# maxwellsh/DIGDriver

Hardware: NVIDIA B200
Metric: genome_bases_scanned_per_s (higher is better)
Workload: dtype u8 bases -> int32 counts; f64 p-values

## Files before the change

### digdriver_b200/_lib.py

```python
import ctypes
import os

_PKG_DIR = os.path.dirname(os.path.abspath(__file__))
LIB_PATH = os.environ.get("DIG_LIB_PATH") or os.path.join(_PKG_DIR, "libdigb200.so")

_c = ctypes
_P = _c.c_void_p
_I64 = _c.c_int64
_I = _c.c_int
_U64 = _c.c_uint64
_D = _c.c_double

SIGNATURES = {
    "dig_version": (_I, []),
    "dig_last_error": (_c.c_char_p, []),
    "dig_device_sm_count": (_I, []),
    "dig_packed_words": (_I64, [_I64]),
    "dig_nmask_words": (_I64, [_I64]),
    "dig_pack_genome": (_I, [_P, _I64, _P, _P, _P, _P]),
    "dig_scan_workspace_bytes": (_I64, [_I64]),
    "dig_count_contexts": (_I, [_P, _P, _I64, _P, _P, _P, _P, _P, _P, _I64, _I, _I, _P, _P, _P, _P]),
    "dig_count_contexts_fused53": (_I, [_P, _P, _I64, _P, _P, _P, _P, _P, _I64, _P, _P, _P, _P, _P, _P]),
    "dig_narrow_counts_u16": (_I, [_P, _I64, _P, _P, _P]),
    "dig_peer_broadcast": (_I, [_P, _I64, _P, _I, _P]),
    "dig_nmask_fill_runs": (_I, [_P, _I64, _P, _I64, _I64, _P]),
    "dig_nmask_summary": (_I, [_P, _I64, _I64, _P, _P]),
    "dig_tabulate_capacity": (_I64, [_I64]),
    "dig_tabulate_elements_workspace_bytes": (_I64, [_I64]),
    "dig_tabulate_genes_workspace_bytes": (_I64, [_I64]),
    "dig_synth_genome": (_I, [_P, _I64, _I64, _U64, _I, _P]),
    "dig_mutation_contexts": (_I, [_P, _P, _I64, _P, _P, _P, _P, _P, _I64, _I, _I, _P, _P]),
    "dig_substitution_counts": (_I, [_P, _P, _I64, _I, _I, _P, _P]),
    "dig_count_hits": (_I, [_P, _P, _P, _P, _I64, _P, _P, _I64, _P, _P]),
    "dig_tabulate_elements": (_I, [_P, _P, _P, _P, _I64, _P, _P, _P, _P, _I64, _P, _P, _P, _I64, _I64, _P,
                                   _I64, _I64, _I64, _P, _P, _I, _P]),
    "dig_site_counts": (_I, [_P, _P, _I64, _I64, _I, _P, _P]),
    "dig_tabulate_genes": (_I, [_P, _P, _P, _I64, _P, _P, _I64, _I64, _I64, _P, _P, _P, _P]),
    "dig_element_transfer": (_I, [_P, _P, _P, _P, _P, _I64, _I64, _I, _P, _P, _P, _P, _P, _P, _P, _I64, _I, _P,
                                  _P, _P, _I, _I, _P, _P, _P, _P, _P, _P, _P, _P, _P, _P]),
    "dig_nb_pvalue_greater_midp": (_I, [_P, _P, _P, _I64, _P, _P]),
    "dig_nb_burden_test": (_I, [_P, _P, _P, _P, _I64, _P, _P, _P]),
    "dig_fisher_combine2": (_I, [_P, _P, _I64, _P, _P]),
    "dig_sequence_freq": (_I, [_P, _P, _I, _P, _P]),
    "dig_size_ratio": (_I, [_P, _P, _I64, _P, _P]),
    "dig_gene_scale_sums": (_I, [_P, _P, _P, _P, _P, _P, _I64, _I64, _P, _P]),
    "dig_gene_burden_test": (_I, [_P, _P, _P, _P, _P, _P, _I64, _P, _D, _D, _P, _P]),
    "dig_gene_dnds_sel": (_I, [_P, _P, _P, _P, _I64, _P, _P]),
    "dig_selection_coefficient": (_I, [_P, _P, _P, _P, _P, _I64, _P, _P, _P]),
    "dig_window_denominators": (_I, [_P, _P, _I64, _P, _P, _P]),
    "dig_site_test": (_I, [_P, _P, _P, _P, _P, _I64, _I64, _I, _P, _P, _P, _P, _P, _P, _P, _D, _P, _P, _P, _P, _P]),
    "dig_region_prob_norm": (_I, [_P, _P, _I64, _I, _P, _P]),
    "dig_position_obs": (_I, [_P, _I64, _P, _P, _P, _P, _P, _I64, _I, _I, _I, _P, _I64, _P, _P]),
    "dig_position_test": (_I, [_P, _P, _I64, _P, _P, _P, _P, _P, _I64, _I, _I, _P, _P, _P, _P, _I, _P, _P, _P, _P,
                               _P, _P, _P]),
    "dig_nb_pvalue_exact": (_I, [_P, _P, _P, _I64, _P, _P]),
    "dig_nb_pvalue_variant": (_I, [_I, _P, _P, _P, _P, _I64, _P, _P]),
    "dig_loglik": (_I, [_I, _P, _P, _P, _I64, _P, _P]),
    "dig_gene_llr_test": (_I, [_I, _P, _P, _P, _P, _P, _P, _I64, _P, _P]),
    "dig_element_region_counts": (_I, [_P, _P, _P, _P, _P, _I64, _I64, _I, _P, _P, _P, _I64, _I, _P, _P, _P, _P]),
    "dig_element_psum": (_I, [_P, _P, _P, _I64, _P, _P, _P]),
    "dig_overlap_count": (_I, [_P, _P, _P, _I64, _P, _P, _I64, _P, _P]),
    "dig_overlap_fill": (_I, [_P, _P, _P, _I64, _P, _P, _I64, _P, _P, _P, _P]),
    "dig_cds_substitution_table": (_I, [_P, _P, _I64, _P, _P, _I, _P, _P, _P, _P, _P, _I64, _P, _I, _P, _I, _P, _P,
                                        _P, _P]),
    "dig_annotate_snvs": (_I, [_P, _P, _I64, _P, _P, _I, _P, _P, _P, _P, _P, _I64, _P, _I, _P, _I, _P, _P, _P, _P,
                               _I64, _P, _P, _P]),
}



class ScanOpts(ctypes.Structure):
    _fields_ = [("workspace_d", _c.c_void_p), ("workspace_bytes", _c.c_int64), ("variant", _c.c_int32),
                ("totals_limit_kb", _c.c_uint32), ("tile_window", _c.c_int64), ("n_peer_counts3", _c.c_int32),
                ("nsum_offset_words", _c.c_int32), ("peer_counts3_d", _c.c_void_p * 8), ("mc_counts3_d", _c.c_void_p)]


SCAN_AUTO, SCAN_PER_BASE, SCAN_HEX_PLAIN, SCAN_HEX = 0, 1, 2, 3

_lib = None

KERNELS_PER_CALL = {
    "dig_pack_genome": 1, "dig_count_contexts": 1, "dig_count_contexts_fused53": 1, "dig_synth_genome": 1, "dig_mutation_contexts": 1,
    "dig_substitution_counts": 1, "dig_count_hits": 1, "dig_tabulate_elements": 3, "dig_tabulate_genes": 2, "dig_site_counts": 1,
    "dig_element_transfer": 1, "dig_nb_pvalue_greater_midp": 1, "dig_nb_burden_test": 1, "dig_fisher_combine2": 1,
    "dig_sequence_freq": 1, "dig_size_ratio": 1, "dig_gene_scale_sums": 1, "dig_gene_burden_test": 2,
    "dig_window_denominators": 1, "dig_site_test": 1, "dig_gene_dnds_sel": 1, "dig_selection_coefficient": 1, "dig_region_prob_norm": 1, "dig_position_obs": 1, "dig_position_test": 1, "dig_nb_pvalue_exact": 1,
    "dig_nb_pvalue_variant": 1, "dig_loglik": 1, "dig_gene_llr_test": 1, "dig_overlap_count": 1, "dig_overlap_fill": 1,
    "dig_element_region_counts": 1, "dig_element_psum": 1, "dig_narrow_counts_u16": 1, "dig_peer_broadcast": 1, "dig_nmask_fill_runs": 1,
    "dig_nmask_summary": 1, "dig_cds_substitution_table": 1, "dig_annotate_snvs": 1,
}
launch_count = 0


class DigError(RuntimeError):
    pass


def load():
    global _lib
    if _lib is not None:
        return _lib
    if not os.path.exists(LIB_PATH):
        raise DigError(
            "libdigb200.so not found at %s: the CUDA extension is required (no CPU fallback). "
            "Build it with `python -m digdriver_b200.build`." % LIB_PATH)
    lib = ctypes.CDLL(LIB_PATH)
    for name, (res, args) in SIGNATURES.items():
        fn = getattr(lib, name)
        fn.restype = res
        fn.argtypes = args
    _lib = lib
    return lib


def check(rc, what=""):
    if rc != 0:
        msg = load().dig_last_error()
        raise DigError("%s failed with code %d: %s" % (what or "libdigb200 call", rc, (msg or b"").decode()))


def call(name, *args):
    global launch_count
    fn = getattr(load(), name)
    check(fn(*args), name)
    launch_count += KERNELS_PER_CALL.get(name, 0)
```

### digdriver_b200/csrc/mutctx.cu

```cuda
#include "dig_common.cuh"

namespace {

__global__ void __launch_bounds__(256) mutctx_kernel(
    const uint32_t *__restrict__ p2, const uint32_t *__restrict__ nmask, int64_t last_p, int64_t last_m,
    const int64_t *__restrict__ chrom_off, const int64_t *__restrict__ chrom_len,
    const int32_t *__restrict__ mut_chrom, const int64_t *__restrict__ mut_start,
    const uint8_t *__restrict__ mut_ref, int64_t n_mut, int n_up, int n_down, int32_t *__restrict__ ctx_out)
{
    const int klen = n_up + n_down + 1;
    const int64_t stride = (int64_t)gridDim.x * blockDim.x;
    for (int64_t i = (int64_t)blockIdx.x * blockDim.x + threadIdx.x; i < n_mut; i += stride) {
        const int32_t c = mut_chrom[i];
        const int64_t p = mut_start[i];
        const int64_t L = __ldg(chrom_len + c);
        const int64_t off = __ldg(chrom_off + c);
        int32_t ctx = -1;
        if (p - n_up >= 0 && p + n_down < L) {
            const int64_t f = off + p - n_up;
            const int64_t w = f >> 4, m = f >> 5;
            const unsigned long long pk = ((unsigned long long)__ldg(p2 + w) << 32) | __ldg(p2 + (w < last_p ? w + 1 : last_p));
            const unsigned long long mk = ((unsigned long long)__ldg(nmask + m) << 32) | __ldg(nmask + (m < last_m ? m + 1 : last_m));
            const uint32_t key = (uint32_t)(pk >> (64 - 2 * ((int)(f & 15) + klen))) & ((1u << (2 * klen)) - 1u);
            const uint32_t bad = (uint32_t)(mk >> (64 - ((int)(f & 31) + klen))) & ((1u << klen) - 1u);
            const uint32_t base = (key >> (2 * n_down)) & 3u;
            const bool base_n = ((bad >> n_down) & 1u) != 0u;
            auto mismatch = [&](int64_t row) -> bool {
                const uint32_t ref = mut_ref[row];
                return ref > 3u || base_n || base != ref;
            };
            bool dropped = mismatch(i);
            for (int64_t j = i - 1; !dropped && j >= 0 && mut_chrom[j] == c && mut_start[j] == p; --j)
                dropped = mismatch(j);
            if (!dropped && bad == 0u) ctx = (int32_t)key;
        }
        ctx_out[i] = ctx;
    }
}

__global__ void __launch_bounds__(256) subst_hist_kernel(const int32_t *__restrict__ ctx,
                                                         const uint8_t *__restrict__ alt, int64_t n, int n_down,
                                                         int n_bins, unsigned long long *__restrict__ counts)
{
    extern __shared__ unsigned int sh[];
    for (int k = threadIdx.x; k < n_bins; k += blockDim.x) sh[k] = 0u;
    __syncthreads();
    const int64_t stride = (int64_t)gridDim.x * blockDim.x;
    for (int64_t i = (int64_t)blockIdx.x * blockDim.x + threadIdx.x; i < n; i += stride) {
        const int32_t c = ctx[i];
        const uint32_t a = alt[i];
        if (c < 0 || a > 3u) continue;
        const uint32_t ref = ((uint32_t)c >> (2 * n_down)) & 3u;
        if (a == ref) continue;
        atomicAdd(sh + 3 * c + (int)(a > ref ? a - 1u : a), 1u);
    }
    __syncthreads();
    for (int k = threadIdx.x; k < n_bins; k += blockDim.x)
        if (sh[k]) atomicAdd(counts + k, (unsigned long long)sh[k]);
}

}

extern "C" int dig_substitution_counts(const int32_t *ctx_d, const uint8_t *alt_d, int64_t n, int n_up, int n_down,
                                       unsigned long long *counts_d, void *stream)
{
    DIG_CHECK_ARG(n >= 0, "negative size");
    DIG_CHECK_ARG(n_up >= 0 && n_down >= 0 && n_up + n_down <= 5, "unsupported context size");
    DIG_CHECK_ARG(counts_d != nullptr, "null pointer");
    const int n_bins = 3 << (2 * (n_up + n_down + 1));
    cudaStream_t st = (cudaStream_t)stream;
    DIG_CUDA(cudaMemsetAsync(counts_d, 0, (size_t)n_bins * sizeof(unsigned long long), st));
    if (n == 0) return DIG_OK;
    DIG_CHECK_ARG(ctx_d && alt_d, "null pointer");
    int64_t blocks = (n + 255) / 256;
    const int64_t cap = (int64_t)dig::sm_count() * 4;
    if (blocks > cap) blocks = cap;
    subst_hist_kernel<<<(unsigned)blocks, 256, (size_t)n_bins * sizeof(unsigned int), st>>>(ctx_d, alt_d, n, n_down,
                                                                                          n_bins, counts_d);
    DIG_CHECK_LAUNCH();
    return DIG_OK;
}

extern "C" int dig_mutation_contexts(const uint32_t *packed2_d, const uint32_t *nmask_d, int64_t n_bases,
                                     const int64_t *chrom_off_d, const int64_t *chrom_len_d,
                                     const int32_t *mut_chrom_d, const int64_t *mut_start_d,
                                     const uint8_t *mut_ref_d, int64_t n_mut, int n_up, int n_down,
                                     int32_t *ctx_out_d, void *stream)
{
    DIG_CHECK_ARG(n_mut >= 0 && n_bases >= 0, "negative size");
    DIG_CHECK_ARG(n_up >= 0 && n_down >= 0 && n_up + n_down <= 14, "unsupported context size");
    if (n_mut == 0) return DIG_OK;
    DIG_CHECK_ARG(packed2_d && nmask_d && chrom_off_d && chrom_len_d && mut_chrom_d && mut_start_d && mut_ref_d &&
                      ctx_out_d,
                  "null pointer");
    int64_t blocks = (n_mut + 255) / 256;
    const int64_t cap = (int64_t)dig::sm_count() * 32;
    if (blocks > cap) blocks = cap;
    mutctx_kernel<<<(unsigned)blocks, 256, 0, (cudaStream_t)stream>>>(
        packed2_d, nmask_d, (((n_bases + 31) >> 5) << 1) - 1, ((n_bases + 31) >> 5) - 1, chrom_off_d, chrom_len_d,
        mut_chrom_d, mut_start_d, mut_ref_d, n_mut, n_up, n_down, ctx_out_d);
    DIG_CHECK_LAUNCH();
    return DIG_OK;
}
```

### digdriver_b200/kernels.py

```python
import numpy as np
import torch

from . import _lib


def _stream(device, stream=None):
    st = stream if stream is not None else torch.cuda.current_stream(device)
    return st.cuda_stream


def _dev(x, dtype, device):
    if isinstance(x, torch.Tensor):
        return x.to(device=device, dtype=dtype).contiguous()
    return torch.from_numpy(np.ascontiguousarray(x)).to(device=device, dtype=dtype)


def _ptr(t):
    return t.data_ptr() if t is not None else None


def _tile_hint(reg_start, reg_end, tile_window):
    if tile_window is not None:
        return int(tile_window)
    if isinstance(reg_start, torch.Tensor) or isinstance(reg_end, torch.Tensor):
        return 0
    s, e = np.asarray(reg_start), np.asarray(reg_end)
    if s.size == 0:
        return 0
    w = int(e.flat[0]) - int(s.flat[0])
    return w if w > 0 and bool(np.all(e - s == w)) else 0


def _scan_opts(dev, n_reg, variant, totals_limit_kb, workspace, tile_window=0, peer_rows=None, mc_rows=None, genome=None):
    import ctypes
    if workspace is None and n_reg > 0:
        nbytes = int(_lib.load().dig_scan_workspace_bytes(int(n_reg)))
        workspace = torch.empty(nbytes, dtype=torch.uint8, device=dev)
    opts = _lib.ScanOpts(workspace.data_ptr() if workspace is not None else None,
                         workspace.numel() if workspace is not None else 0, int(variant), int(totals_limit_kb),
                         int(tile_window))
    if peer_rows:
        assert len(peer_rows) <= 8, "at most 8 peers"
        opts.n_peer_counts3 = len(peer_rows)
        for i, a in enumerate(peer_rows):
            opts.peer_counts3_d[i] = int(a)
        opts.mc_counts3_d = int(mc_rows) if mc_rows else None
    if genome is not None and getattr(genome, "nsum", None) is not None:
        assert genome.nsum.data_ptr() == genome.nmask.data_ptr() + 4 * genome.nsum_offset
        opts.nsum_offset_words = genome.nsum_offset
    return opts, ctypes.byref(opts), workspace


def peer_broadcast(src, dst_addrs, stream=None):
    import ctypes
    dev = src.device
    arr = (ctypes.c_void_p * len(dst_addrs))(*[int(a) for a in dst_addrs])
    with torch.cuda.device(dev):
        _lib.call("dig_peer_broadcast", src.data_ptr(), src.numel() * src.element_size(), arr, len(dst_addrs), _stream(dev, stream))


def scan_workspace(genome_or_device, n_reg):
    dev = getattr(genome_or_device, "device", genome_or_device)
    return torch.empty(int(_lib.load().dig_scan_workspace_bytes(int(n_reg))), dtype=torch.uint8, device=dev)


def count_contexts(genome, reg_chrom, reg_start, reg_end, n_up=1, n_down=1, strand=None,
                   want_totals=False, out=None, totals=None, stream=None, variant=_lib.SCAN_AUTO,
                   totals_limit_kb=0, workspace=None, tile_window=None, peer_rows=None, mc_rows=None):
    dev = genome.device
    rc = _dev(reg_chrom, torch.int32, dev)
    rs = _dev(reg_start, torch.int64, dev)
    re = _dev(reg_end, torch.int64, dev)
    st = _dev(strand, torch.int8, dev) if strand is not None else None
    n = rc.numel()
    K = 4 ** (n_up + n_down + 1)
    if out is None:
        out = torch.empty((n, K), dtype=torch.int32, device=dev)
    if want_totals and totals is None:
        totals = torch.zeros(K, dtype=torch.int64, device=dev)
    lane_bank = (n_up, n_down) in ((2, 2), (1, 1)) and st is None and variant == _lib.SCAN_AUTO
    opts, opts_ref, workspace = _scan_opts(dev, n if lane_bank else 0, variant, totals_limit_kb,
                                           workspace if lane_bank else None,
                                           _tile_hint(reg_start, reg_end, tile_window) if lane_bank else 0,
                                           peer_rows, mc_rows, genome)
    with torch.cuda.device(dev):
        _lib.call("dig_count_contexts", genome.packed2.data_ptr(), genome.nmask.data_ptr(), genome.n_bases,
                  genome.chrom_off_d.data_ptr(), genome.chrom_len_d.data_ptr(), rc.data_ptr(), rs.data_ptr(),
                  re.data_ptr(), _ptr(st), n, int(n_up), int(n_down), out.data_ptr(), _ptr(totals), opts_ref,
                  _stream(dev, stream))
    if lane_bank and n > 0:
        _lib.launch_count += 1
    return out, totals


def count_contexts_fused53(genome, reg_chrom, reg_start, reg_end, want_totals=False, out5=None, out3=None,
                           totals5=None, totals3=None, stream=None, variant=_lib.SCAN_AUTO, totals_limit_kb=0,
                           workspace=None, tile_window=None, peer_rows=None, mc_rows=None):
    dev = genome.device
    rc = _dev(reg_chrom, torch.int32, dev)
    rs = _dev(reg_start, torch.int64, dev)
    re = _dev(reg_end, torch.int64, dev)
    n = rc.numel()
    if out5 is None:
        out5 = torch.empty((n, 1024), dtype=torch.int32, device=dev)
    if out3 is None:
        out3 = torch.empty((n, 64), dtype=torch.int32, device=dev)
    if want_totals and totals5 is None:
        totals5 = torch.zeros(1024, dtype=torch.int64, device=dev)
        totals3 = torch.zeros(64, dtype=torch.int64, device=dev)
    lane_bank = variant == _lib.SCAN_AUTO
    opts, opts_ref, workspace = _scan_opts(dev, n if lane_bank else 0, variant, totals_limit_kb,
                                           workspace if lane_bank else None,
                                           _tile_hint(reg_start, reg_end, tile_window) if lane_bank else 0,
                                           peer_rows, mc_rows, genome)
    with torch.cuda.device(dev):
        _lib.call("dig_count_contexts_fused53", genome.packed2.data_ptr(), genome.nmask.data_ptr(), genome.n_bases,
                  genome.chrom_off_d.data_ptr(), genome.chrom_len_d.data_ptr(), rc.data_ptr(), rs.data_ptr(),
                  re.data_ptr(), n, out5.data_ptr(), out3.data_ptr(), _ptr(totals5), _ptr(totals3), opts_ref,
                  _stream(dev, stream))
    if lane_bank and n > 0:
        _lib.launch_count += 1
    return out5, out3, totals5, totals3


def mutation_contexts(genome, mut_chrom, mut_start, mut_ref, n_up=1, n_down=1, stream=None):
    dev = genome.device
    mc = _dev(mut_chrom, torch.int32, dev)
    ms = _dev(mut_start, torch.int64, dev)
    mr = _dev(mut_ref, torch.uint8, dev)
    out = torch.empty(mc.numel(), dtype=torch.int32, device=dev)
    with torch.cuda.device(dev):
        _lib.call("dig_mutation_contexts", genome.packed2.data_ptr(), genome.nmask.data_ptr(), genome.n_bases,
                  genome.chrom_off_d.data_ptr(), genome.chrom_len_d.data_ptr(), mc.data_ptr(), ms.data_ptr(),
                  mr.data_ptr(), mc.numel(), int(n_up), int(n_down), out.data_ptr(), _stream(dev, stream))
    return out


def nb_pvalue_greater_midp(k, alpha, p, device="cuda:0", stream=None):
    dev = torch.device(device)
    kd, ad, pd_ = (_dev(x, torch.float64, dev) for x in (k, alpha, p))
    out = torch.empty_like(kd)
    with torch.cuda.device(dev):
        _lib.call("dig_nb_pvalue_greater_midp", kd.data_ptr(), ad.data_ptr(), pd_.data_ptr(), kd.numel(),
                  out.data_ptr(), _stream(dev, stream))
    return out


def nb_burden_test(k, alpha, theta, pi, device="cuda:0", want_exp=True, stream=None):
    dev = torch.device(device)
    kd, ad, td, fd = (_dev(x, torch.float64, dev) for x in (k, alpha, theta, pi))
    pval = torch.empty_like(kd)
    exp = torch.empty_like(kd) if want_exp else None
    with torch.cuda.device(dev):
        _lib.call("dig_nb_burden_test", kd.data_ptr(), ad.data_ptr(), td.data_ptr(), fd.data_ptr(), kd.numel(),
                  _ptr(exp), pval.data_ptr(), _stream(dev, stream))
    return exp, pval


def fisher_combine2(p1, p2, device="cuda:0", stream=None):
    dev = torch.device(device)
    a, b = _dev(p1, torch.float64, dev), _dev(p2, torch.float64, dev)
    out = torch.empty_like(a)
    with torch.cuda.device(dev):
        _lib.call("dig_fisher_combine2", a.data_ptr(), b.data_ptr(), a.numel(), out.data_ptr(), _stream(dev, stream))
    return out


def _table_capacity(n_pairs):
    return int(_lib.load().dig_tabulate_capacity(int(n_pairs)))


def _check_status(status, what, sink=None):
    if sink is not None:
        sink.append((status, what))
        return
    code = int(status.item())
    if code == 1:
        raise _lib.DigError("%s: hash table overflow" % what)
    if code == 2:
        raise KeyError("%s: an element overlaps a window that is not in region_params "
                       "(the reference raises KeyError on the same input)" % what)
    if code == 3:
        raise _lib.DigError("%s: element window span exceeds the shared-memory bitmap" % what)
    if code != 0:
        raise _lib.DigError("%s: status %d" % (what, code))


def check_deferred(sink):
    pending, sink[:] = list(sink), []
    for status, what in pending:
        _check_status(status, what)


def tabulate_elements(blk_kstart, blk_kend, blk_elt, mut_kstart, mut_kend, mut_sample, mut_isindel,
                      n_elt, n_sample, max_muts_per_sample=10 ** 9, max_per_elt_per_sample=3 * 10 ** 9,
                      device="cuda:0", stream=None, sample_rows_mode=False, return_table=False, max_hits=None,
                      status_sink=None):
    dev = torch.device(device)
    bks = np.asarray(blk_kstart, dtype=np.int64)
    order = np.argsort(bks, kind="stable")
    bks = bks[order]
    bke = np.asarray(blk_kend, dtype=np.int64)[order]
    belt = np.asarray(blk_elt, dtype=np.int32)[order]
    pmax = np.maximum.accumulate(bke) if len(bke) else bke
    t = {k: _dev(v, dt, dev) for k, v, dt in (
        ("bks", bks, torch.int64), ("bke", bke, torch.int64), ("pmax", pmax, torch.int64), ("belt", belt, torch.int32),
        ("mks", mut_kstart, torch.int64), ("mke", mut_kend, torch.int64), ("ms", mut_sample, torch.int32),
        ("mi", mut_isindel, torch.uint8))}
    n_blk, n_mut = len(bks), t["mks"].numel()
    sptr = _stream(dev, stream)
    with torch.cuda.device(dev):
        if max_hits is None:
            n_hits = torch.zeros(1, dtype=torch.int64, device=dev)
            _lib.call("dig_count_hits", t["bks"].data_ptr(), t["bke"].data_ptr(), t["pmax"].data_ptr(),
                      t["belt"].data_ptr(), n_blk, t["mks"].data_ptr(), t["mke"].data_ptr(), n_mut, n_hits.data_ptr(), sptr)
            max_hits = int(n_hits.item())
        cap = _table_capacity(max_hits)
        keys = torch.empty(cap, dtype=torch.int64, device=dev)
        snv = torch.empty(cap, dtype=torch.int32, device=dev)
        ind = torch.empty(cap, dtype=torch.int32, device=dev)
        sample_tot = torch.empty(max(n_sample, 1), dtype=torch.int64, device=dev)
        obs = torch.empty((max(n_elt, 1), 3), dtype=torch.int64, device=dev)
        status = torch.zeros(1, dtype=torch.int32, device=dev)
        _lib.call("dig_tabulate_elements", t["bks"].data_ptr(), t["bke"].data_ptr(), t["pmax"].data_ptr(),
                  t["belt"].data_ptr(), n_blk, t["mks"].data_ptr(), t["mke"].data_ptr(), t["ms"].data_ptr(),
                  t["mi"].data_ptr(), n_mut, keys.data_ptr(), snv.data_ptr(), ind.data_ptr(), cap, n_sample,
                  sample_tot.data_ptr(), int(min(max_muts_per_sample, 2 ** 62)),
                  int(min(max_per_elt_per_sample, 2 ** 62)), n_elt, obs.data_ptr(), status.data_ptr(),
                  int(bool(sample_rows_mode)), sptr)
        _check_status(status, "dig_tabulate_elements", status_sink)
    if return_table:
        return obs[:n_elt], sample_tot[:n_sample], (keys, snv, ind)
    return obs[:n_elt], sample_tot[:n_sample]


def tabulate_genes(mut_gene, mut_sample, mut_class, n_gene, max_per_gene_per_sample=3 * 10 ** 9,
                   device="cuda:0", stream=None, status_sink=None):
    dev = torch.device(device)
    mg, ms, mc = _dev(mut_gene, torch.int32, dev), _dev(mut_sample, torch.int32, dev), _dev(mut_class, torch.uint8, dev)
    n_mut = mg.numel()
    cap = _table_capacity(n_mut)
    with torch.cuda.device(dev):
        keys = torch.empty(cap, dtype=torch.int64, device=dev)
        cnt = torch.empty((cap, 5), dtype=torch.int32, device=dev)
        obs = torch.empty((max(n_gene, 1), 5), dtype=torch.int64, device=dev)
        nsamp = torch.empty((max(n_gene, 1), 7), dtype=torch.int64, device=dev)
        status = torch.zeros(1, dtype=torch.int32, device=dev)
        _lib.call("dig_tabulate_genes", mg.data_ptr(), ms.data_ptr(), mc.data_ptr(), n_mut, keys.data_ptr(),
                  cnt.data_ptr(), cap, int(min(max_per_gene_per_sample, 2 ** 62)), n_gene, obs.data_ptr(),
                  nsamp.data_ptr(), status.data_ptr(), _stream(dev, stream))
        _check_status(status, "dig_tabulate_genes", status_sink)
    return obs[:n_gene], nsamp[:n_gene]


def element_transfer(elt_chrom, elt_strand, blk_ptr, blk_start, blk_end, window, win_map_off, win_map,
                     win_counts, y_pred, std, y_true, flag, d_pr, blk_counts=None, L_elt=None,
                     device="cuda:0", stream=None, max_span=None, status_sink=None):
    dev = torch.device(device)
    ec, es = _dev(elt_chrom, torch.int32, dev), _dev(elt_strand, torch.int8, dev)
    bp, bs, be = (_dev(x, torch.int64, dev) for x in (blk_ptr, blk_start, blk_end))
    wmo, wm = _dev(win_map_off, torch.int64, dev), _dev(win_map, torch.int32, dev)
    wc = _dev(win_counts, torch.int32, dev)
    yp, sd, yt = (_dev(x, torch.float64, dev).reshape(-1, wc.shape[0]) for x in (y_pred, std, y_true))
    fl = _dev(np.asarray(flag).astype(np.uint8) if not isinstance(flag, torch.Tensor) else flag.to(torch.uint8),
              torch.uint8, dev).reshape(-1, wc.shape[0])
    dp = _dev(d_pr, torch.float64, dev).reshape(-1, 192)
    n_cohort = dp.shape[0]
    assert yp.shape[0] == n_cohort and sd.shape[0] == n_cohort and yt.shape[0] == n_cohort and fl.shape[0] == n_cohort
    n_elt = ec.numel()
    n_win = wc.shape[0]
    if blk_counts is not None:
        bc, Le, n_col = _dev(blk_counts, torch.int32, dev), None, 1
    else:
        Le = _dev(L_elt, torch.float64, dev)
        Le = Le.reshape(n_elt, 192, -1)
        bc, n_col = None, Le.shape[2]
    if max_span is None:
        max_span = element_max_span(bp, bs, be, window)
    out = {
        "MU": torch.empty((n_cohort, n_elt), dtype=torch.float64, device=dev),
        "SIGMA": torch.empty((n_cohort, n_elt), dtype=torch.float64, device=dev),
        "R_OBS": torch.empty((n_cohort, n_elt), dtype=torch.float64, device=dev),
        "FLAG": torch.empty((n_cohort, n_elt), dtype=torch.uint8, device=dev),
        "R_SIZE": torch.empty(n_elt, dtype=torch.int64, device=dev),
        "ELT_SIZE": torch.empty(n_elt, dtype=torch.int64, device=dev),
        "P": torch.empty((n_cohort, n_elt, n_col), dtype=torch.float64, device=dev),
        "N_WIN": torch.empty(n_elt, dtype=torch.int32, device=dev),
    }
    status = torch.zeros(1, dtype=torch.int32, device=dev)
    with torch.cuda.device(dev):
        _lib.call("dig_element_transfer", ec.data_ptr(), es.data_ptr(), bp.data_ptr(), bs.data_ptr(), be.data_ptr(),
                  n_elt, int(window), int(wmo.numel()) - 1, wmo.data_ptr(), wm.data_ptr(), wc.data_ptr(), yp.data_ptr(),
                  sd.data_ptr(), yt.data_ptr(), fl.data_ptr(), n_win, n_cohort, dp.data_ptr(), _ptr(bc), _ptr(Le), n_col, max_span,
                  out["MU"].data_ptr(), out["SIGMA"].data_ptr(), out["R_OBS"].data_ptr(), out["FLAG"].data_ptr(),
                  out["R_SIZE"].data_ptr(), out["ELT_SIZE"].data_ptr(), out["P"].data_ptr(),
                  out["N_WIN"].data_ptr(), status.data_ptr(), _stream(dev, stream))
        _check_status(status, "dig_element_transfer", status_sink)
    return out


def element_max_span(blk_ptr, blk_start, blk_end, window):
    def host(x):
        return x.cpu().numpy() if isinstance(x, torch.Tensor) else np.asarray(x)
    bp_h, bs_h, be_h = host(blk_ptr).astype(np.int64), host(blk_start).astype(np.int64), host(blk_end).astype(np.int64)
    n_elt = len(bp_h) - 1
    max_span = 1
    if n_elt > 0 and len(bs_h):
        lo = np.floor_divide(bs_h, window)
        hi = -np.floor_divide(-be_h, window)
        owner = np.repeat(np.arange(n_elt), np.diff(bp_h))
        wmin = np.full(n_elt, np.iinfo(np.int64).max)
        wmax = np.full(n_elt, np.iinfo(np.int64).min)
        np.minimum.at(wmin, owner, lo)
        np.maximum.at(wmax, owner, hi)
        has = wmax > wmin
        if has.any():
            max_span = int((wmax[has] - wmin[has]).max())
    return max_span


def build_window_map(win_chrom_idx, win_start, window, n_chrom):
    wc = np.asarray(win_chrom_idx, dtype=np.int64)
    wn = np.asarray(win_start, dtype=np.int64) // int(window)
    per = np.zeros(n_chrom, dtype=np.int64)
    if len(wc):
        np.maximum.at(per, wc, wn + 1)
    off = np.zeros(n_chrom + 1, dtype=np.int64)
    off[1:] = np.cumsum(per)
    wmap = np.full(int(off[-1]), -1, dtype=np.int32)
    wmap[off[wc] + wn] = np.arange(len(wc), dtype=np.int32)
    return off, wmap


def substitution_counts(ctx, alt, n_up=1, n_down=1, stream=None, out=None):
    dev = ctx.device
    al = _dev(alt, torch.uint8, dev)
    if out is None:
        out = torch.empty(3 * 4 ** (n_up + n_down + 1), dtype=torch.int64, device=dev)
    assert out.dtype == torch.int64 and out.is_contiguous() and out.numel() == 3 * 4 ** (n_up + n_down + 1)
    with torch.cuda.device(dev):
        _lib.call("dig_substitution_counts", ctx.data_ptr(), al.data_ptr(), ctx.numel(), int(n_up), int(n_down),
                  out.data_ptr(), _stream(dev, stream))
    return out


def sequence_freq(subst_counts, ctx_totals, stream=None):
    dev = subst_counts.device
    n_ctx = ctx_totals.numel()
    out = torch.empty(3 * n_ctx, dtype=torch.float64, device=dev)
    with torch.cuda.device(dev):
        _lib.call("dig_sequence_freq", subst_counts.data_ptr(), ctx_totals.data_ptr(), n_ctx, out.data_ptr(),
                  _stream(dev, stream))
    return out


GENE_OUT_ROWS = (["EXP_" + c for c in ("SYN", "MIS", "NONS", "SPL", "TRUNC", "NONSYN")] +
                 ["PVAL_%s_BURDEN" % c for c in ("SYN", "MIS", "NONS", "SPL", "TRUNC", "NONSYN")] +
                 ["PVAL_%s_BURDEN_SAMPLE" % c for c in ("SYN", "MIS", "NONS", "SPL", "TRUNC", "NONSYN")] +
                 ["EXP_INDEL", "PVAL_INDEL_BURDEN", "PVAL_MUT_BURDEN", "ALPHA", "THETA", "THETA_INDEL", "Pi_INDEL",
                  "Pi_TRUNC", "Pi_NONSYN"])


def size_ratio(num, den, stream=None):
    dev = num.device
    assert num.dtype == torch.int64 and den.dtype == torch.int64 and num.is_contiguous() and den.is_contiguous()
    assert num.numel() == den.numel()
    out = torch.empty(num.shape, dtype=torch.float64, device=dev)
    with torch.cuda.device(dev):
        _lib.call("dig_size_ratio", num.data_ptr(), den.data_ptr(), num.numel(), out.data_ptr(), _stream(dev, stream))
    return out


def gene_scale_sums(mu, sigma, P, pi_indel, obs, cgc_mask=None, tp53=-1, stream=None):
    dev = mu.device
    sums = torch.empty(3, dtype=torch.float64, device=dev)
    cg = _dev(cgc_mask, torch.uint8, dev) if cgc_mask is not None else None
    with torch.cuda.device(dev):
        _lib.call("dig_gene_scale_sums", mu.data_ptr(), sigma.data_ptr(), P.data_ptr(), pi_indel.data_ptr(),
                  obs.data_ptr(), _ptr(cg), int(tp53), mu.numel(), sums.data_ptr(), _stream(dev, stream))
    return sums


def gene_burden_test(mu, sigma, P, pi_indel, obs, nsamp, sums, n_syn, scale_factor=None, stream=None):
    dev = mu.device
    E = mu.numel()
    out = torch.empty((len(GENE_OUT_ROWS), E), dtype=torch.float64, device=dev)
    with torch.cuda.device(dev):
        _lib.call("dig_gene_burden_test", mu.data_ptr(), sigma.data_ptr(), P.data_ptr(), pi_indel.data_ptr(),
                  obs.data_ptr(), nsamp.data_ptr(), E, sums.data_ptr(), float("nan") if n_syn is None else float(n_syn),
                  float("nan") if scale_factor is None else float(scale_factor), out.data_ptr(), _stream(dev, stream))
    return out


def site_counts(site_elt, site_sub, n_elt, n_sub=192, device="cuda:0", stream=None):
    dev = torch.device(device)
    se, ss = _dev(site_elt, torch.int32, dev), _dev(site_sub, torch.int32, dev)
    out = torch.empty((max(n_elt, 1), n_sub), dtype=torch.int64, device=dev)
    with torch.cuda.device(dev):
        _lib.call("dig_site_counts", se.data_ptr(), ss.data_ptr(), se.numel(), n_elt, n_sub, out.data_ptr(),
                  _stream(dev, stream))
    return out[:n_elt]


def nb_pvalue_exact(k, alpha, p, device="cuda:0", stream=None):
    dev = torch.device(device)
    kk, aa, pp = (_dev(x, torch.float64, dev).contiguous() for x in (k, alpha, p))
    out = torch.empty_like(kk)
    with torch.cuda.device(dev):
        _lib.call("dig_nb_pvalue_exact", kk.data_ptr(), aa.data_ptr(), pp.data_ptr(), kk.numel(), out.data_ptr(),
                  _stream(dev, stream))
    return out


def position_bins(genome, reg_chrom, reg_start, reg_end, n_up, n_down, binsize):
    rc = np.asarray(reg_chrom, dtype=np.int64)
    rs = np.asarray(reg_start, dtype=np.int64).copy()
    re = np.asarray(reg_end, dtype=np.int64)
    L = np.asarray(genome.chrom_len, dtype=np.int64)[rc]
    rs[rs < n_up] = n_up
    first = np.minimum(rs, L)
    last = np.minimum(re + n_down, L) - n_down
    n_pos = np.maximum(last - first, 0)
    n_bin = -(-n_pos // binsize)
    ptr = np.zeros(len(rc) + 1, dtype=np.int64)
    ptr[1:] = np.cumsum(n_bin)
    return first, n_pos, ptr


def position_test(genome, reg_chrom, reg_start, reg_end, mu, sigma, s_prob, mut_chrom, mut_start, n_up=2, n_down=2,
                  binsize=1, normed=True, want=("pt", "exp", "pos"), stream=None):
    dev = genome.device
    rc = _dev(reg_chrom, torch.int32, dev)
    rs = _dev(reg_start, torch.int64, dev)
    re = _dev(reg_end, torch.int64, dev)
    n_reg = rc.numel()
    K = 4 ** (n_up + n_down + 1)
    sp = _dev(s_prob, torch.float64, dev).contiguous()
# ... 305 lines not shown
```

### include/dig_b200.h

```cpp
#ifndef DIG_B200_H
#define DIG_B200_H

#include <stdint.h>

#ifdef __cplusplus
extern "C" {
#endif

#define DIG_OK 0
#define DIG_ERR_ARG (-1)
#define DIG_ERR_CUDA (-2)
#define DIG_ERR_RANGE (-3)
#define DIG_ERR_UNSUPPORTED (-4)

int dig_version(void);
const char *dig_last_error(void);
int dig_device_sm_count(void);

int64_t dig_packed_words(int64_t n_bases);
int64_t dig_nmask_words(int64_t n_bases);
int dig_pack_genome(const uint8_t *ascii_d, int64_t n_bases, uint32_t *packed2_d, uint32_t *nmask_d,
                    unsigned long long *n_other_d, void *stream);

#define DIG_SCAN_AUTO 0
#define DIG_SCAN_PER_BASE 1
#define DIG_SCAN_HEX_PLAIN 2
#define DIG_SCAN_HEX 3
typedef struct dig_scan_opts {
    void *workspace_d;
    int64_t workspace_bytes;
    int32_t variant;
    uint32_t totals_limit_kb;
    int64_t tile_window;
    int32_t n_peer_counts3;
    int32_t nsum_offset_words;
    void *peer_counts3_d[8];
    void *mc_counts3_d;
} dig_scan_opts;
int64_t dig_scan_workspace_bytes(int64_t n_reg);

int dig_count_contexts(const uint32_t *packed2_d, const uint32_t *nmask_d, int64_t n_bases,
                       const int64_t *chrom_off_d, const int64_t *chrom_len_d,
                       const int32_t *reg_chrom_d, const int64_t *reg_start_d, const int64_t *reg_end_d,
                       const int8_t *reg_strand_d, int64_t n_reg, int n_up, int n_down,
                       int32_t *counts_d, unsigned long long *totals_d, const dig_scan_opts *opts, void *stream);

int dig_count_contexts_fused53(const uint32_t *packed2_d, const uint32_t *nmask_d, int64_t n_bases,
                               const int64_t *chrom_off_d, const int64_t *chrom_len_d,
                               const int32_t *reg_chrom_d, const int64_t *reg_start_d, const int64_t *reg_end_d,
                               int64_t n_reg, int32_t *counts5_d, int32_t *counts3_d,
                               unsigned long long *totals5_d, unsigned long long *totals3_d,
                               const dig_scan_opts *opts, void *stream);

int dig_narrow_counts_u16(const int32_t *counts_d, int64_t n_values, uint16_t *out_d, int32_t *status_d, void *stream);

int dig_nmask_fill_runs(const int64_t *runs_d, int64_t n_runs, uint32_t *nmask_d, int64_t word0, int64_t n_words, void *stream);

int dig_nmask_summary(const uint32_t *nmask_d, int64_t word0, int64_t n_words, uint32_t *nsum_d, void *stream);

int dig_peer_broadcast(const void *src_d, int64_t nbytes, void *const *dst_d, int n_dst, void *stream);

int dig_mutation_contexts(const uint32_t *packed2_d, const uint32_t *nmask_d, int64_t n_bases,
                          const int64_t *chrom_off_d, const int64_t *chrom_len_d,
                          const int32_t *mut_chrom_d, const int64_t *mut_start_d, const uint8_t *mut_ref_d,
                          int64_t n_mut, int n_up, int n_down, int32_t *ctx_out_d, void *stream);

int dig_substitution_counts(const int32_t *ctx_d, const uint8_t *alt_d, int64_t n, int n_up, int n_down,
                            unsigned long long *counts_d, void *stream);

int64_t dig_tabulate_capacity(int64_t n_pairs);
int64_t dig_tabulate_elements_workspace_bytes(int64_t n_pairs);
int64_t dig_tabulate_genes_workspace_bytes(int64_t n_mut);
int dig_count_hits(const int64_t *blk_kstart_d, const int64_t *blk_kend_d, const int64_t *blk_pmax_d,
                   const int32_t *blk_elt_d, int64_t n_blk, const int64_t *mut_kstart_d,
                   const int64_t *mut_kend_d, int64_t n_mut, unsigned long long *n_hits_d, void *stream);
int dig_tabulate_elements(const int64_t *blk_kstart_d, const int64_t *blk_kend_d, const int64_t *blk_pmax_d,
                          const int32_t *blk_elt_d, int64_t n_blk, const int64_t *mut_kstart_d,
                          const int64_t *mut_kend_d, const int32_t *mut_sample_d, const uint8_t *mut_isindel_d,
                          int64_t n_mut, unsigned long long *tab_key_d, uint32_t *tab_snv_d,
                          uint32_t *tab_indel_d, int64_t capacity, int64_t n_sample,
                          unsigned long long *sample_tot_d, int64_t max_muts_per_sample,
                          int64_t max_per_elt_per_sample, int64_t n_elt, int64_t *obs_d, int32_t *status_d,
                          int sample_rows_mode, void *stream);

int dig_site_counts(const int32_t *site_elt_d, const int32_t *site_sub_d, int64_t n_site, int64_t n_elt, int n_sub,
                    unsigned long long *L_d, void *stream);

int dig_tabulate_genes(const int32_t *mut_gene_d, const int32_t *mut_sample_d, const uint8_t *mut_class_d,
                       int64_t n_mut, unsigned long long *tab_key_d, uint32_t *tab_cnt_d, int64_t capacity,
                       int64_t max_per_gene_per_sample, int64_t n_gene, int64_t *obs_d, int64_t *nsamp_d,
                       int32_t *status_d, void *stream);

int dig_element_transfer(const int32_t *elt_chrom_d, const int8_t *elt_strand_d, const int64_t *blk_ptr_d,
                         const int64_t *blk_start_d, const int64_t *blk_end_d, int64_t n_elt, int64_t window,
                         int n_chrom, const int64_t *win_map_off_d, const int32_t *win_map_d,
                         const int32_t *win_counts_d, const double *y_pred_d, const double *std_d, const double *y_true_d,
                         const uint8_t *flag_d, int64_t n_win, int n_cohort, const double *d_pr_d,
                         const int32_t *blk_counts_d, const double *L_elt_d, int n_col, int max_span_windows,
                         double *mu_d, double *sigma_d, double *r_obs_d, uint8_t *flag_out_d, int64_t *r_size_d,
                         int64_t *elt_size_d, double *p_out_d, int32_t *n_win_out_d, int32_t *status_d,
                         void *stream);

int dig_nb_pvalue_greater_midp(const double *k_d, const double *alpha_d, const double *p_d, int64_t n,
                               double *pval_out_d, void *stream);
int dig_nb_burden_test(const double *k_d, const double *alpha_d, const double *theta_d, const double *pi_d,
                       int64_t n, double *exp_out_d, double *pval_out_d, void *stream);
int dig_fisher_combine2(const double *p1_d, const double *p2_d, int64_t n, double *out_d, void *stream);

int dig_sequence_freq(const unsigned long long *subst_counts_d, const unsigned long long *ctx_totals_d, int n_ctx,
                      double *freq_d, void *stream);
int dig_size_ratio(const int64_t *num_d, const int64_t *den_d, int64_t n, double *out_d, void *stream);
int dig_gene_scale_sums(const double *mu_d, const double *sigma_d, const double *p_d, const double *pi_indel_d,
                        const int64_t *obs_d, const uint8_t *cgc_mask_d, int64_t tp53, int64_t n_gene,
                        double *sums_d, void *stream);
int dig_gene_burden_test(const double *mu_d, const double *sigma_d, const double *p_d, const double *pi_indel_d,
                         const int64_t *obs_d, const int64_t *nsamp_d, int64_t n_gene, const double *sums_d,
                         double n_syn, double scale_factor, double *out_d, void *stream);

int dig_gene_dnds_sel(const double *alpha_d, const double *theta_d, const double *pi6_d, const double *obs6_d,
                      int64_t n_gene, double *out_d, void *stream);
int dig_selection_coefficient(const double *obs_d, const double *exp_d, const double *alpha_d, const double *theta_d,
                              const double *pi_d, int64_t n, double *sel_d, double *pval_d, void *stream);

int dig_window_denominators(const int32_t *win_counts_d, const double *d_pr_d, int64_t n_win, double *denom_plus_d,
                            double *denom_minus_d, void *stream);
int dig_site_test(const int32_t *site_chrom_d, const int64_t *site_start_d, const uint8_t *site_sub_d,
                  const int8_t *site_strand_d, const double *site_k_d, int64_t n_site, int64_t window, int n_chrom,
                  const int64_t *win_map_off_d, const int32_t *win_map_d, const double *y_pred_d, const double *std_d,
                  const double *denom_plus_d, const double *denom_minus_d, const double *d_pr_d, double cj,
                  double *p_out_d, double *exp_out_d, double *pval_out_d, int32_t *status_d, void *stream);

int dig_region_prob_norm(const int32_t *counts_d, const double *s_prob_d, int64_t n_reg, int n_ctx, double *norm_d,
                         void *stream);
int dig_position_obs(const int64_t *mut_key_d, int64_t n_mut, const int64_t *chrom_off_d, const int64_t *chrom_len_d,
                     const int32_t *reg_chrom_d, const int64_t *reg_start_d, const int64_t *reg_end_d, int64_t n_reg,
                     int n_up, int n_down, int binsize, const int64_t *bin_ptr_d, int64_t n_bin, int32_t *obs_d,
                     void *stream);
int dig_position_test(const uint32_t *packed2_d, const uint32_t *nmask_d, int64_t n_bases, const int64_t *chrom_off_d,
                      const int64_t *chrom_len_d, const int32_t *reg_chrom_d, const int64_t *reg_start_d,
                      const int64_t *reg_end_d, int64_t n_reg, int n_up, int n_down, const double *s_prob_d,
                      const double *norm_d, const double *mu_d, const double *sigma_d, int binsize,
                      const int64_t *bin_ptr_d, const int32_t *obs_d, double *pval_d, double *pt_d, double *exp_d,
                      double *pos_d, void *stream);
int dig_nb_pvalue_exact(const double *k_d, const double *alpha_d, const double *p_d, int64_t n, double *pval_out_d,
                        void *stream);

#define DIG_NB_GREATER 0
#define DIG_NB_GREATER_MIDP 1
#define DIG_NB_LESS 2
#define DIG_NB_LESS_MIDP 3
#define DIG_NB_EXACT 4
#define DIG_NB_MIDP 5
int dig_nb_pvalue_variant(int mode, const double *k_d, const double *alpha_d, const double *p_d, const double *mu_d,
                          int64_t n, double *pval_out_d, void *stream);

#define DIG_LL_NB 0
#define DIG_LL_POIS 1
#define DIG_LL_GAMMA 2
int dig_loglik(int kind, const double *x_d, const double *a_d, const double *b_d, int64_t n, double *out_d, void *stream);

#define DIG_LLR_NB 0
#define DIG_LLR_GAMMA_POISSON 1
int dig_gene_llr_test(int model, const double *alpha_d, const double *theta_d, const double *pi3_d, const double *obs3_d,
                      const double *mrfold_d, const double *t_syn_d, int64_t n, double *out_d, void *stream);

int dig_overlap_count(const int64_t *blk_kstart_d, const int64_t *blk_kend_d, const int64_t *blk_pmax_d, int64_t n_blk,
                      const int64_t *mut_kstart_d, const int64_t *mut_kend_d, int64_t n_mut, int64_t *n_pairs_d,
                      void *stream);
int dig_overlap_fill(const int64_t *blk_kstart_d, const int64_t *blk_kend_d, const int64_t *blk_pmax_d, int64_t n_blk,
                     const int64_t *mut_kstart_d, const int64_t *mut_kend_d, int64_t n_mut, const int64_t *pair_off_d,
                     int64_t *pair_mut_d, int64_t *pair_blk_d, void *stream);

int dig_element_region_counts(const int32_t *elt_chrom_d, const int8_t *elt_strand_d, const int64_t *blk_ptr_d,
                              const int64_t *blk_start_d, const int64_t *blk_end_d, int64_t n_elt, int64_t window,
                              int n_chrom, const int64_t *win_map_off_d, const int32_t *win_map_d,
                              const int32_t *win_counts_d, int64_t n_win, int max_span_windows, int64_t *region_counts_d, int32_t *n_win_out_d,
                              int32_t *status_d, void *stream);

int dig_element_psum(const double *L_d, const int64_t *region_counts_d, const double *d_pr_d, int64_t n_elt,
                     double *p_out_d, double *denom_out_d, void *stream);

#define DIG_CDS_SYNONYMOUS 0
#define DIG_CDS_MISSENSE 1
#define DIG_CDS_NONSENSE 2
#define DIG_CDS_ESSENTIAL_SPLICE 3
#define DIG_CDS_STOP_LOSS 5
#define DIG_CDS_NO_HIT 255
#define DIG_CDS_FLAG_LENGTH 1
#define DIG_CDS_FLAG_N 2
#define DIG_CDS_FLAG_STOP 4
#define DIG_CDS_ERR_BLOCKS 1
#define DIG_CDS_ERR_RANGE 2
#define DIG_CDS_ERR_ORDER 4
#define DIG_CDS_MAX_BLOCKS 2048
#define DIG_CDS_MAX_SPLICE_OFFSETS 8
int dig_cds_substitution_table(const uint32_t *packed2_d, const uint32_t *nmask_d, int64_t n_bases,
                               const int64_t *chrom_off_d, const int64_t *chrom_len_d, int n_chrom,
                               const int32_t *gene_chrom_d, const int8_t *gene_strand_d, const int64_t *blk_ptr_d,
                               const int64_t *blk_start_d, const int64_t *blk_end_d, int64_t n_gene,
                               const int32_t *donor, int n_donor, const int32_t *acceptor, int n_acceptor,
                               double *L_d, int32_t *flags_d, int32_t *status_d, void *stream);
int dig_annotate_snvs(const uint32_t *packed2_d, const uint32_t *nmask_d, int64_t n_bases,
                      const int64_t *chrom_off_d, const int64_t *chrom_len_d, int n_chrom,
                      const int32_t *gene_chrom_d, const int8_t *gene_strand_d, const int64_t *blk_ptr_d,
                      const int64_t *blk_start_d, const int64_t *blk_end_d, int64_t n_gene,
                      const int32_t *donor, int n_donor, const int32_t *acceptor, int n_acceptor,
                      const int64_t *mut_pos_d, const uint8_t *mut_alt_d, const int64_t *pair_mut_d,
                      const int32_t *pair_gene_d, int64_t n_pair, uint8_t *class_out_d, int32_t *status_d,
                      void *stream);

int dig_synth_genome(uint8_t *ascii_d, int64_t g0, int64_t n, uint64_t seed, int n_frac16, void *stream);

#ifdef __cplusplus
}
#endif
#endif
```

Before: 2828 billion.

## Skip N-mask loads via block summary in mutctx; replicate and vectorise subst histogram

The mutation-context kernel now consults a coarse N-summary bitmap (2 bits per 128-base block) and only loads the full N-mask words when a block may contain Ns. The substitution histogram kernel uses per-warp replicated shared-memory histograms, 512 threads, and vectorised int4/uchar4 loads to cut shared atomic contention. The intent is fewer memory loads and less atomic serialisation, at the cost of extra reduction work and a changed C ABI (a new trailing argument).

Result: faster. 2870 billion (median of 6 runs) (+1.5%).

```diff
diff --git a/digdriver_b200/_lib.py b/digdriver_b200/_lib.py
--- a/digdriver_b200/_lib.py
+++ b/digdriver_b200/_lib.py
@@ -29,7 +29,7 @@
     "dig_tabulate_elements_workspace_bytes": (_I64, [_I64]),
     "dig_tabulate_genes_workspace_bytes": (_I64, [_I64]),
     "dig_synth_genome": (_I, [_P, _I64, _I64, _U64, _I, _P]),
-    "dig_mutation_contexts": (_I, [_P, _P, _I64, _P, _P, _P, _P, _P, _I64, _I, _I, _P, _P]),
+    "dig_mutation_contexts": (_I, [_P, _P, _I64, _P, _P, _P, _P, _P, _I64, _I, _I, _P, _P, _c.c_int32]),
     "dig_substitution_counts": (_I, [_P, _P, _I64, _I, _I, _P, _P]),
     "dig_count_hits": (_I, [_P, _P, _P, _P, _I64, _P, _P, _I64, _P, _P]),
     "dig_tabulate_elements": (_I, [_P, _P, _P, _P, _I64, _P, _P, _P, _P, _I64, _P, _P, _P, _I64, _I64, _P,
diff --git a/digdriver_b200/csrc/mutctx.cu b/digdriver_b200/csrc/mutctx.cu
--- a/digdriver_b200/csrc/mutctx.cu
+++ b/digdriver_b200/csrc/mutctx.cu
@@ -3,8 +3,8 @@
 namespace {
 
 __global__ void __launch_bounds__(256) mutctx_kernel(
-    const uint32_t *__restrict__ p2, const uint32_t *__restrict__ nmask, int64_t last_p, int64_t last_m,
-    const int64_t *__restrict__ chrom_off, const int64_t *__restrict__ chrom_len,
+    const uint32_t *__restrict__ p2, const uint32_t *__restrict__ nmask, const uint32_t *__restrict__ nsum,
+    int64_t last_p, int64_t last_m, const int64_t *__restrict__ chrom_off, const int64_t *__restrict__ chrom_len,
     const int32_t *__restrict__ mut_chrom, const int64_t *__restrict__ mut_start,
     const uint8_t *__restrict__ mut_ref, int64_t n_mut, int n_up, int n_down, int32_t *__restrict__ ctx_out)
 {
@@ -20,9 +20,19 @@
             const int64_t f = off + p - n_up;
             const int64_t w = f >> 4, m = f >> 5;
             const unsigned long long pk = ((unsigned long long)__ldg(p2 + w) << 32) | __ldg(p2 + (w < last_p ? w + 1 : last_p));
-            const unsigned long long mk = ((unsigned long long)__ldg(nmask + m) << 32) | __ldg(nmask + (m < last_m ? m + 1 : last_m));
+            bool any_n = true;
+            if (nsum != nullptr) {
+                const int64_t b0 = f >> 7, b1 = (f + klen - 1) >> 7;
+                const uint32_t s0 = __ldg(nsum + (b0 >> 4)) >> (2 * (int)(b0 & 15));
+                const uint32_t s1 = __ldg(nsum + (b1 >> 4)) >> (2 * (int)(b1 & 15));
+                any_n = ((s0 | s1) & 1u) != 0u;
+            }
+            uint32_t bad = 0u;
+            if (any_n) {
+                const unsigned long long mk = ((unsigned long long)__ldg(nmask + m) << 32) | __ldg(nmask + (m < last_m ? m + 1 : last_m));
+                bad = (uint32_t)(mk >> (64 - ((int)(f & 31) + klen))) & ((1u << klen) - 1u);
+            }
             const uint32_t key = (uint32_t)(pk >> (64 - 2 * ((int)(f & 15) + klen))) & ((1u << (2 * klen)) - 1u);
-            const uint32_t bad = (uint32_t)(mk >> (64 - ((int)(f & 31) + klen))) & ((1u << klen) - 1u);
             const uint32_t base = (key >> (2 * n_down)) & 3u;
             const bool base_n = ((bad >> n_down) & 1u) != 0u;
             auto mismatch = [&](int64_t row) -> bool {
@@ -38,25 +48,45 @@
     }
 }
 
-__global__ void __launch_bounds__(256) subst_hist_kernel(const int32_t *__restrict__ ctx,
-                                                         const uint8_t *__restrict__ alt, int64_t n, int n_down,
-                                                         int n_bins, unsigned long long *__restrict__ counts)
+constexpr int HIST_THREADS = 512;
+
+__global__ void __launch_bounds__(HIST_THREADS) subst_hist_kernel(const int32_t *__restrict__ ctx,
+                                                                  const uint8_t *__restrict__ alt, int64_t n, int n_down,
+                                                                  int n_bins, int copies,
+                                                                  unsigned long long *__restrict__ counts)
 {
     extern __shared__ unsigned int sh[];
-    for (int k = threadIdx.x; k < n_bins; k += blockDim.x) sh[k] = 0u;
+    for (int k = threadIdx.x; k < n_bins * copies; k += blockDim.x) sh[k] = 0u;
     __syncthreads();
+    unsigned int *hist = sh + ((int)threadIdx.x >> 5) % copies * n_bins;
+    auto add = [&](int32_t c, uint32_t a) {
+        if (c < 0 || a > 3u) return;
+        const uint32_t ref = ((uint32_t)c >> (2 * n_down)) & 3u;
+        if (a == ref) return;
+        atomicAdd(hist + 3 * c + (int)(a > ref ? a - 1u : a), 1u);
+    };
+    const int64_t tid = (int64_t)blockIdx.x * blockDim.x + threadIdx.x;
     const int64_t stride = (int64_t)gridDim.x * blockDim.x;
-    for (int64_t i = (int64_t)blockIdx.x * blockDim.x + threadIdx.x; i < n; i += stride) {
-        const int32_t c = ctx[i];
-        const uint32_t a = alt[i];
-        if (c < 0 || a > 3u) continue;
-        const uint32_t ref = ((uint32_t)c >> (2 * n_down)) & 3u;
-        if (a == ref) continue;
-        atomicAdd(sh + 3 * c + (int)(a > ref ? a - 1u : a), 1u);
+    int64_t done = 0;
+    if ((reinterpret_cast<uintptr_t>(ctx) & 15u) == 0 && (reinterpret_cast<uintptr_t>(alt) & 3u) == 0) {
+        const int64_t n4 = n >> 2;
+        for (int64_t i = tid; i < n4; i += stride) {
+            const int4 c = __ldg(reinterpret_cast<const int4 *>(ctx) + i);
+            const uchar4 a = __ldg(reinterpret_cast<const uchar4 *>(alt) + i);
+            add(c.x, a.x);
+            add(c.y, a.y);
+            add(c.z, a.z);
+            add(c.w, a.w);
+        }
+        done = n4 << 2;
     }
+    for (int64_t i = done + tid; i < n; i += stride) add(ctx[i], alt[i]);
     __syncthreads();
-    for (int k = threadIdx.x; k < n_bins; k += blockDim.x)
-        if (sh[k]) atomicAdd(counts + k, (unsigned long long)sh[k]);
+    for (int k = threadIdx.x; k < n_bins; k += blockDim.x) {
+        unsigned int v = 0u;
+        for (int q = 0; q < copies; ++q) v += sh[q * n_bins + k];
+        if (v) atomicAdd(counts + k, (unsigned long long)v);
+    }
 }
 
 }
@@ -72,11 +102,13 @@
     DIG_CUDA(cudaMemsetAsync(counts_d, 0, (size_t)n_bins * sizeof(unsigned long long), st));
     if (n == 0) return DIG_OK;
     DIG_CHECK_ARG(ctx_d && alt_d, "null pointer");
-    int64_t blocks = (n + 255) / 256;
-    const int64_t cap = (int64_t)dig::sm_count() * 4;
+    int64_t blocks = (n + 4 * HIST_THREADS - 1) / (4 * HIST_THREADS);
+    const int64_t cap = (int64_t)dig::sm_count();
     if (blocks > cap) blocks = cap;
-    subst_hist_kernel<<<(unsigned)blocks, 256, (size_t)n_bins * sizeof(unsigned int), st>>>(ctx_d, alt_d, n, n_down,
-                                                                                          n_bins, counts_d);
+    int copies = (int)((48 * 1024) / ((size_t)n_bins * sizeof(unsigned int)));
+    copies = copies < 1 ? 1 : (copies > HIST_THREADS / 32 ? HIST_THREADS / 32 : copies);
+    subst_hist_kernel<<<(unsigned)blocks, HIST_THREADS, (size_t)copies * n_bins * sizeof(unsigned int), st>>>(
+        ctx_d, alt_d, n, n_down, n_bins, copies, counts_d);
     DIG_CHECK_LAUNCH();
     return DIG_OK;
 }
@@ -85,8 +117,9 @@
                                      const int64_t *chrom_off_d, const int64_t *chrom_len_d,
                                      const int32_t *mut_chrom_d, const int64_t *mut_start_d,
                                      const uint8_t *mut_ref_d, int64_t n_mut, int n_up, int n_down,
-                                     int32_t *ctx_out_d, void *stream)
+                                     int32_t *ctx_out_d, void *stream, int32_t nsum_offset_words)
 {
+    DIG_CHECK_ARG(nsum_offset_words >= 0, "negative nsum_offset_words");
     DIG_CHECK_ARG(n_mut >= 0 && n_bases >= 0, "negative size");
     DIG_CHECK_ARG(n_up >= 0 && n_down >= 0 && n_up + n_down <= 14, "unsupported context size");
     if (n_mut == 0) return DIG_OK;
@@ -97,7 +130,7 @@
     const int64_t cap = (int64_t)dig::sm_count() * 32;
     if (blocks > cap) blocks = cap;
     mutctx_kernel<<<(unsigned)blocks, 256, 0, (cudaStream_t)stream>>>(
-        packed2_d, nmask_d, (((n_bases + 31) >> 5) << 1) - 1, ((n_bases + 31) >> 5) - 1, chrom_off_d, chrom_len_d,
+        packed2_d, nmask_d, nsum_offset_words > 0 ? nmask_d + nsum_offset_words : nullptr, (((n_bases + 31) >> 5) << 1) - 1, ((n_bases + 31) >> 5) - 1, chrom_off_d, chrom_len_d,
         mut_chrom_d, mut_start_d, mut_ref_d, n_mut, n_up, n_down, ctx_out_d);
     DIG_CHECK_LAUNCH();
     return DIG_OK;
diff --git a/digdriver_b200/kernels.py b/digdriver_b200/kernels.py
--- a/digdriver_b200/kernels.py
+++ b/digdriver_b200/kernels.py
@@ -129,10 +129,14 @@
     ms = _dev(mut_start, torch.int64, dev)
     mr = _dev(mut_ref, torch.uint8, dev)
     out = torch.empty(mc.numel(), dtype=torch.int32, device=dev)
+    nsum_off = 0
+    if getattr(genome, "nsum", None) is not None:
+        assert genome.nsum.data_ptr() == genome.nmask.data_ptr() + 4 * genome.nsum_offset
+        nsum_off = genome.nsum_offset
     with torch.cuda.device(dev):
         _lib.call("dig_mutation_contexts", genome.packed2.data_ptr(), genome.nmask.data_ptr(), genome.n_bases,
                   genome.chrom_off_d.data_ptr(), genome.chrom_len_d.data_ptr(), mc.data_ptr(), ms.data_ptr(),
-                  mr.data_ptr(), mc.numel(), int(n_up), int(n_down), out.data_ptr(), _stream(dev, stream))
+                  mr.data_ptr(), mc.numel(), int(n_up), int(n_down), out.data_ptr(), _stream(dev, stream), nsum_off)
     return out
 
 
diff --git a/include/dig_b200.h b/include/dig_b200.h
--- a/include/dig_b200.h
+++ b/include/dig_b200.h
@@ -63,7 +63,8 @@
 int dig_mutation_contexts(const uint32_t *packed2_d, const uint32_t *nmask_d, int64_t n_bases,
                           const int64_t *chrom_off_d, const int64_t *chrom_len_d,
                           const int32_t *mut_chrom_d, const int64_t *mut_start_d, const uint8_t *mut_ref_d,
-                          int64_t n_mut, int n_up, int n_down, int32_t *ctx_out_d, void *stream);
+                          int64_t n_mut, int n_up, int n_down, int32_t *ctx_out_d, void *stream,
+                          int32_t nsum_offset_words);
 
 int dig_substitution_counts(const int32_t *ctx_d, const uint8_t *alt_d, int64_t n, int n_up, int n_down,
                             unsigned long long *counts_d, void *stream);
```
